# bcgsc/RNA-Bloom

Hardware: AMD Instinct MI355X
Metric: k-mers/sec hashed+inserted into Bloom dBG (k=25, 50M 150bp reads) (higher is better)
Workload: dtype u64

## Files before the change

### rna-bloom_amd/csrc/rb_capi.hip

```cpp
#include <math.h>
#include <stdarg.h>
#include <stdlib.h>
#include <string.h>
#include <time.h>

#include <algorithm>
#include <new>
#include <vector>

#include <functional>
#include <string>
#include <thread>

#include <fcntl.h>
#include <unistd.h>
#include <zlib.h>

#include "rb_pipeline.hpp"

using namespace rb;

namespace {

__global__ void k_popcount_bits(const uint32_t *__restrict__ w, size_t n_words, unsigned long long *out) {
// ... 652 lines not shown
            size_t m = std::min(chunk, n - done);
            g->keys0.reserve(m * 8); g->vals0.reserve(m * 4);
            RB_HIP(hipMemcpyAsync(g->keys0.p, h0 + done, m * 8, hipMemcpyHostToDevice, s));
            hipLaunchKernelGGL(k_iota, dim3(blocks_for((int64_t)m)), dim3(TPB), 0, s, g->vals0.as<uint32_t>(), m);
            run_pipeline(g, m, mode, g->ordinal, 0, nullptr);
            g->ordinal += m;
            done += m;
        }
        RB_HIP(hipStreamSynchronize(s));
    });
}

}
namespace {
__global__ void k_debug_probe(uint32_t *words, uint64_t n_words, uint32_t per_thread, int mode, uint64_t salt, unsigned long long *sink) {
    const uint64_t t = (uint64_t)blockIdx.x * blockDim.x + threadIdx.x;
    uint64_t x = (t + salt) * 0x9E3779B97F4A7C15ull + 0x632BE59BD9B4E019ull;
    uint32_t acc = 0;
    for (uint32_t i = 0; i < per_thread; ++i) {
        x ^= x >> 30; x *= 0xBF58476D1CE4E5B9ull; x ^= x >> 27; x *= 0x94D049BB133111EBull; x ^= x >> 31;
        uint32_t *w = &words[(uint64_t)(((unsigned __int128)x * n_words) >> 64)];
        acc |= mode ? atomicXor(w, 0x80808080u) : atomicOr(w, 0u);
    }
    if (acc == 0x12345678u) atomicAdd(sink, 1ull);
}
}
extern "C" {
int rb_debug_probe_cbf(rb_graph *g, int mode, float *ms_out) {
    return guarded([&] {
        RB_REQUIRE(g && g->cbf && ms_out, "rb_debug_probe_cbf: bad argument");
        rb::WriteLock wl(g->rw);
        RB_HIP(hipSetDevice(g->p.device));
        hipStream_t s = g->stream;
        g->devctr.reserve(DEVCTR_BYTES);
        rb::Event e0, e1;
        RB_HIP(hipEventCreate(&e0.e)); RB_HIP(hipEventCreate(&e1.e));
        RB_HIP(hipStreamSynchronize(s));
        RB_HIP(hipEventRecord(e0, s));
        for (int pass = 0; pass < 2; ++pass)
            hipLaunchKernelGGL(k_debug_probe, dim3(65536), dim3(256), 0, s, reinterpret_cast<uint32_t *>(g->cbf), (uint64_t)(g->cbf_alloc / 4), 16u, mode, 0ull, g->devctr.as<unsigned long long>());
        RB_HIP(hipEventRecord(e1, s));
        RB_HIP(hipEventSynchronize(e1));
        RB_HIP(hipEventElapsedTime(ms_out, e0, e1));
    });
}

int rb_debug_scan_u32(int device, const uint32_t *in, size_t n, uint32_t *out, int misalign) {
    DevBuf a, b, t;
    return guarded([&] {
        RB_REQUIRE((in && out) || n == 0, "rb_debug_scan_u32: null array");
        RB_REQUIRE(misalign >= 0 && misalign < 16, "rb_debug_scan_u32: misalign in 0..15");
        RB_HIP(hipSetDevice(device));
        a.reserve((n + 8) * 4); b.reserve((n + 8) * 4); t.reserve(scan_temp_bytes(n));
        uint32_t *di = a.as<uint32_t>() + (misalign & 3), *dout = b.as<uint32_t>() + ((misalign >> 2) & 3);
        if (n) RB_HIP(hipMemcpy(di, in, n * 4, hipMemcpyHostToDevice));
        exclusive_scan_u32(t.p, t.cap, di, dout, n, nullptr);
        RB_HIP(hipGetLastError());
        RB_HIP(hipDeviceSynchronize());
        if (n) RB_HIP(hipMemcpy(out, dout, n * 4, hipMemcpyDeviceToHost));
    });
}
int rb_debug_sort_pairs(int device, uint64_t *keys, void *vals, int vals64, size_t n, int lo_begin, int lo_end, int hi_begin, int hi_end) {
    DevBuf k0, k1, v0, v1, t;
    return guarded([&] {
        RB_REQUIRE(keys || n == 0, "rb_debug_sort_pairs: null keys");
        RB_REQUIRE(!(vals64 && hi_begin >= 0), "rb_debug_sort_pairs: two ranges with 32-bit values only");
        RB_HIP(hipSetDevice(device));
        if (n == 0) return;
        const size_t vb = vals64 ? 8 : 4;
        k0.reserve(n * 8); k1.reserve(n * 8);
        if (vals) { v0.reserve(n * vb); v1.reserve(n * vb); RB_HIP(hipMemcpy(v0.p, vals, n * vb, hipMemcpyHostToDevice)); }
        RB_HIP(hipMemcpy(k0.p, keys, n * 8, hipMemcpyHostToDevice));
        t.reserve(vals64 ? sort_pairs32_temp_bytes(n) : sort_pairs_temp_bytes(n));
        if (vals64) sort_pairs_u64_u64(t.p, t.cap, k0.as<uint64_t>(), k1.as<uint64_t>(), v0.as<uint64_t>(), v1.as<uint64_t>(), n, lo_begin, lo_end, nullptr);
        else if (hi_begin >= 0) sort_pairs_u64_u32_2r(t.p, t.cap, k0.as<uint64_t>(), k1.as<uint64_t>(), v0.as<uint32_t>(), v1.as<uint32_t>(), n, lo_begin, lo_end, hi_begin, hi_end, nullptr);
        else if (vals) sort_pairs_u64_u32(t.p, t.cap, k0.as<uint64_t>(), k1.as<uint64_t>(), v0.as<uint32_t>(), v1.as<uint32_t>(), n, lo_begin, lo_end, nullptr);
        else sort_keys_u64(t.p, t.cap, k0.as<uint64_t>(), k1.as<uint64_t>(), n, lo_begin, lo_end, nullptr);
        RB_HIP(hipGetLastError());
        RB_HIP(hipDeviceSynchronize());
        RB_HIP(hipMemcpy(keys, k1.p, n * 8, hipMemcpyDeviceToHost));
        if (vals) RB_HIP(hipMemcpy(vals, v1.p, n * vb, hipMemcpyDeviceToHost));
    });
}
int rb_filter_size(rb_graph *g, int which, int64_t *size, int64_t *nbytes, int *num_hash) {
    if (!g) { set_error("null graph"); return RB_ERR_INVALID; }
    if (which == RB_CBF) {
        if (!g->cbf) { set_error("rb_filter_size: filter %d not initialised", which); return RB_ERR_STATE; }
        if (size) *size = g->cbf_size;
        if (nbytes) *nbytes = g->cbf_hi - g->cbf_lo;
        if (num_hash) *num_hash = g->cbf_h;
        return RB_OK;
    }
    BitFilter *f = bit_filter(g, which);
    if (!f) { set_error("rb_filter_size: unknown filter %d", which); return RB_ERR_INVALID; }
    if (!f->bits) { set_error("rb_filter_size: filter %d not initialised", which); return RB_ERR_STATE; }
    if (size) *size = f->size;
    if (nbytes) *nbytes = f->nbytes;
    if (num_hash) *num_hash = f->num_hash;
    return RB_OK;
}

static int filter_reduce(rb_graph *g, int which, bool fold, unsigned long long *out) {
    return guarded([&] {
        RB_REQUIRE(g && out, "rb_filter_popcount / rb_filter_fold: null argument");
        QueryLease q(g);
        RB_HIP(hipStreamSynchronize(g->stream));
        q.c->b0.reserve(64);
        unsigned long long *acc = q.c->b0.as<unsigned long long>();
        RB_HIP(hipMemsetAsync(acc, 0, 8, q.c->st));
        const uint32_t *words; size_t nw; uint64_t gw0;
        if (which == RB_CBF) {
            if (!g->cbf) { set_error("rb_filter_popcount: filter %d not initialised", which); throw HipError{RB_ERR_STATE}; }
            words = reinterpret_cast<const uint32_t *>(g->cbf); nw = g->cbf_alloc / 4;
            gw0 = (uint64_t)g->cbf_lo / 4u;
        } else {
            BitFilter *f = bit_filter(g, which);
            RB_REQUIRE(f, "rb_filter_popcount: unknown filter %d", which);
            if (!f->bits) { set_error("rb_filter_popcount: filter %d not initialised", which); throw HipError{RB_ERR_STATE}; }
            words = f->bits; nw = f->alloc / 4;
            gw0 = (uint64_t)f->lo / 32u;
        }
        const dim3 grid(std::min<unsigned>(blocks_for((int64_t)nw), 8192u));
        if (fold) hipLaunchKernelGGL(k_fold_words, grid, dim3(TPB), 0, q.c->st, words, nw, gw0, acc);
        else if (which == RB_CBF) hipLaunchKernelGGL(k_count_nonzero_bytes, grid, dim3(TPB), 0, q.c->st, words, nw, acc);
        else hipLaunchKernelGGL(k_popcount_bits, grid, dim3(TPB), 0, q.c->st, words, nw, acc);
        RB_HIP(hipGetLastError());
        unsigned long long v = 0;
        RB_HIP(hipMemcpyAsync(&v, acc, 8, hipMemcpyDeviceToHost, q.c->st));
        RB_HIP(hipStreamSynchronize(q.c->st));
        *out = v;
    });
}
int rb_filter_popcount(rb_graph *g, int which, int64_t *out) {
    unsigned long long v = 0;
    if (!out) { set_error("rb_filter_popcount: null argument"); return RB_ERR_INVALID; }
    int rc = filter_reduce(g, which, false, &v);
    if (rc == RB_OK) *out = (int64_t)v;
    return rc;
}
int rb_filter_fold(rb_graph *g, int which, uint64_t *out) {
    unsigned long long v = 0;
    if (!out) { set_error("rb_filter_fold: null argument"); return RB_ERR_INVALID; }
    int rc = filter_reduce(g, which, true, &v);
    if (rc == RB_OK) *out = (uint64_t)v;
    return rc;
}

int rb_filter_fpr(rb_graph *g, int which, float *out) {
    int64_t pop = 0, size = 0; int h = 0;
    int rc = rb_filter_popcount(g, which, &pop);
    if (rc != RB_OK) return rc;
    rc = rb_filter_size(g, which, &size, nullptr, &h);
    if (rc != RB_OK) return rc;
    if (!out) { set_error("null argument"); return RB_ERR_INVALID; }
    *out = (float)pow((double)pop / (double)size, h);
    return RB_OK;
}

int rb_filter_export(rb_graph *g, int which, void *dst, size_t nbytes) {
    return guarded([&] {
        RB_REQUIRE(g && dst, "rb_filter_export: null argument");
        QueryLease q(g);
        const void *src; size_t have;
        if (which == RB_CBF) { src = g->cbf; have = (size_t)(g->cbf_hi - g->cbf_lo); }
        else {
            BitFilter *f = bit_filter(g, which);
// ... 123 lines not shown
```

### rna-bloom_amd/csrc/rb_group.hip

```cpp
#include <stdlib.h>

#include <algorithm>

#include "rb_pipeline.hpp"

namespace rb {

constexpr uint32_t GR_KEY_TOP = 60;
constexpr uint32_t GR_MAX_GROUP_BITS = 36;
constexpr uint32_t GR_TILE = 4096;
constexpr uint32_t GR_BUCKET_TARGET = 3072;
constexpr uint32_t GR_LOCAL_BITS = 8;
constexpr uint32_t GR_PART_MAX_BITS = 10;

constexpr uint64_t GR_DEAD_KEY = ~0ull;
constexpr uint32_t GR_DEAD_VAL = ~0u;
__device__ __forceinline__ uint32_t gr_digit(uint64_t key, uint32_t shift, uint32_t bits) {
    return (uint32_t)(key >> shift) & ((1u << bits) - 1u);
}
struct GrIdxDev { Mod mod; uint64_t lo, mul; uint32_t top, shift; };
__device__ __forceinline__ uint32_t gr_idx_digit(uint64_t key, const GrIdxDev &ix, uint32_t bits) {
    const uint64_t i = index_of(key, ix.mod) - ix.lo;
    const uint32_t d = min((uint32_t)min(__umul64hi(i, ix.mul), (uint64_t)0xFFFFFFFFull), ix.top);
    return (d >> ix.shift) & ((1u << bits) - 1u);
// ... 51 lines not shown
template <int ITEMS, typename CT>
__device__ __forceinline__ void gr_wave_rank_lds_wide(const uint32_t (&dig)[ITEMS], uint32_t (&rank)[ITEMS], CT *wc, unsigned long long *wm, uint32_t bits,
                                                      uint32_t rows) {
    const uint32_t lane = threadIdx.x & 63u;
#pragma unroll
    for (int r = 0; r < ITEMS; ++r) {
        if ((uint32_t)r < rows) {
            const bool valid = dig[r] != ~0u;
            uint64_t ml = 0;
            uint32_t prior = 0;
            if (valid) {
                __hip_atomic_fetch_or(&wm[dig[r] & 255u], 1ull << lane, __ATOMIC_RELAXED, __HIP_MEMORY_SCOPE_WORKGROUP);
                ml = __hip_atomic_load(&wm[dig[r] & 255u], __ATOMIC_RELAXED, __HIP_MEMORY_SCOPE_WORKGROUP);
                prior = (uint32_t)wc[dig[r]];
            }
            uint64_t m = ml;
            for (uint32_t b = 8; b < bits; ++b) {
                const bool bit = valid && ((dig[r] >> b) & 1u);
                const uint64_t bal = __ballot(bit);
                m &= bit ? bal : ~bal;
            }
            rank[r] = prior + gr_lanes_below(m);
            if (valid && (ml >> lane) == 1ull) __hip_atomic_store(&wm[dig[r] & 255u], 0ull, __ATOMIC_RELAXED, __HIP_MEMORY_SCOPE_WORKGROUP);
            if (valid && (m >> lane) == 1ull) wc[dig[r]] = (CT)(prior + (uint32_t)__popcll(m));
            __builtin_amdgcn_wave_barrier();
        }
    }
}

template <int TPB>
__device__ __forceinline__ uint32_t gr_block_excl_scan(uint32_t v, uint32_t *s_wsum) {
    const uint32_t lane = threadIdx.x & 63u, w = threadIdx.x >> 6;
    uint32_t inc = v;
#pragma unroll
    for (int o = 1; o < 64; o <<= 1) {
        const uint32_t t = __shfl_up(inc, o, 64);
        if ((int)lane >= o) inc += t;
    }
    if (lane == 63u) s_wsum[w] = inc;
    __syncthreads();
    uint32_t base = 0;
#pragma unroll
    for (int i = 0; i < TPB / 64; ++i) {
        const uint32_t t = s_wsum[i];
        if ((uint32_t)i < w) base += t;
    }
    __syncthreads();
    return base + inc - v;
}

template <int TPB, typename CT, typename DT>
__device__ __forceinline__ void gr_digit_offsets(CT *wcnt , DT *dstart , uint32_t nb, uint32_t *s_wsum) {
    constexpr int NW = TPB / 64;
    const uint32_t per = (nb + TPB - 1) / TPB;
    uint32_t tot[4] = {0, 0, 0, 0}, sum = 0;
    for (uint32_t q = 0; q < per; ++q) {
        const uint32_t d = threadIdx.x * per + q;
        if (d < nb) {
            uint32_t run = 0;
#pragma unroll
            for (int w = 0; w < NW; ++w) { const uint32_t t = (uint32_t)wcnt[(uint32_t)w * nb + d]; wcnt[(uint32_t)w * nb + d] = (CT)run; run += t; }
            tot[q] = run; sum += run;
        }
    }
    uint32_t base = gr_block_excl_scan<TPB>(sum, s_wsum);
    for (uint32_t q = 0; q < per; ++q) {
        const uint32_t d = threadIdx.x * per + q;
        if (d < nb) { dstart[d] = (DT)base; base += tot[q]; }
    }
}

__device__ __forceinline__ uint32_t gr_tile_of_block(uint32_t b, uint32_t grid_tiles, int xcd_map) {
    if (!xcd_map) return b;
    return (b & 7u) * (grid_tiles >> 3) + (b >> 3);
}
inline uint32_t gr_grid_for_tiles(uint32_t ntiles) { return ((ntiles + 7u) / 8u) * 8u; }

struct GrTile { uint32_t start, count, hist_base, hist_stride; };
struct GrTiling {
    const GrTile *desc;
    const uint32_t *ntiles_dev;
    uint32_t n, ntiles, grid_tiles;
    int xcd_map;
};
__device__ __forceinline__ bool gr_get_tile(const GrTiling &tl, GrTile &t) {
    const uint32_t i = gr_tile_of_block(blockIdx.x, tl.grid_tiles, tl.xcd_map);
    if (!tl.desc) {
        if (i >= tl.ntiles) return false;
        t.start = i * GR_TILE; t.count = min(GR_TILE, tl.n - t.start); t.hist_base = i; t.hist_stride = tl.ntiles;
        return true;
    }
    if (i >= *tl.ntiles_dev) return false;
    t = tl.desc[i];
    return true;
}

template <int TPB, bool DERIVE = false>
__global__ void __launch_bounds__(TPB) k_part_count(const uint64_t *__restrict__ keys, GrTiling tl, uint32_t shift, uint32_t bits,
                                                    uint32_t *__restrict__ hist, const uint32_t *__restrict__ dead_vals = nullptr,
                                                    GrIdxDev ix = GrIdxDev{Mod{1, 0, 0}, 0, 0, 0, 0}, uint64_t kmul = 0) {
    constexpr int ITEMS = GR_TILE / TPB;
    __shared__ uint32_t s_h[1u << GR_PART_MAX_BITS];
    GrTile t;
    if (!gr_get_tile(tl, t)) return;
    const uint32_t nb = 1u << bits;
    for (uint32_t d = threadIdx.x; d < nb; d += TPB) s_h[d] = 0;
    __syncthreads();
    uint64_t k[ITEMS];
#pragma unroll
    for (int i = 0; i < ITEMS; ++i) {
        const uint32_t j = (uint32_t)i * TPB + threadIdx.x;
        k[i] = j < t.count ? keys[t.start + j] : 0ull;
        if (DERIVE) k[i] = multi_hash(k[i], 1u, kmul);
    }
#pragma unroll
    for (int i = 0; i < ITEMS; ++i) {
        const uint32_t j = (uint32_t)i * TPB + threadIdx.x;
        if (j < t.count && !(dead_vals && k[i] == GR_DEAD_KEY && dead_vals[t.start + j] == GR_DEAD_VAL))
            atomicAdd(&s_h[ix.mul ? gr_idx_digit(k[i], ix, bits) : gr_digit(k[i], shift, bits)], 1u);
    }
    __syncthreads();
    for (uint32_t d = threadIdx.x; d < nb; d += TPB) hist[(size_t)t.hist_base + (size_t)d * t.hist_stride] = s_h[d];
}

template <int TPB, int MAXBITS, bool DERIVE = false>
__global__ void __launch_bounds__(TPB) k_part_scatter(const uint64_t *__restrict__ keys_in, const uint32_t *__restrict__ vals_in, GrTiling tl,
                                                      uint32_t shift, uint32_t bits, const uint32_t *__restrict__ goffs ,
                                                      uint64_t *__restrict__ keys_out, uint32_t *__restrict__ vals_out, uint32_t wide_lds,
                                                      uint32_t skip_dead = 0u, GrIdxDev ix = GrIdxDev{Mod{1, 0, 0}, 0, 0, 0, 0}, uint64_t kmul = 0) {
    constexpr uint32_t ITEMS = GR_TILE / TPB, NW = TPB / 64, SEG = 64 * ITEMS, MAXNB = 1u << MAXBITS;
    __shared__ uint64_t s_keys[GR_TILE];
    __shared__ uint32_t s_vals[GR_TILE];
    __shared__ uint32_t s_cnt[NW * MAXNB / 2 > MAXNB ? NW * MAXNB / 2 : MAXNB];
    __shared__ uint16_t s_dstart[MAXNB];
    __shared__ uint32_t s_wsum[NW];
    constexpr bool NARROW = MAXBITS <= 8;
    static_assert(sizeof(s_vals) >= NW * 256u * sizeof(unsigned long long), "the mask table must fit the staging array");
    unsigned long long *s_wmask = reinterpret_cast<unsigned long long *>(s_vals);
    uint16_t *s_wcnt = reinterpret_cast<uint16_t *>(s_cnt);
    GrTile t;
    if (!gr_get_tile(tl, t)) return;
    const uint32_t nb = 1u << bits;
    const uint32_t w = threadIdx.x >> 6, lane = threadIdx.x & 63u;
    for (uint32_t d = threadIdx.x; d < NW * nb; d += TPB) s_wcnt[d] = 0;
    for (uint32_t d = threadIdx.x; d < NW * (NARROW ? nb : 256u); d += TPB) s_wmask[d] = 0ull;
    uint64_t k[ITEMS];
    uint32_t v[ITEMS], dig[ITEMS], rank[ITEMS];
#pragma unroll
    for (uint32_t r = 0; r < ITEMS; ++r) {
        const uint32_t j = w * SEG + r * 64u + lane;
        bool ok = j < t.count;
        k[r] = ok ? keys_in[t.start + j] : 0ull;
        v[r] = (ok && vals_in) ? vals_in[t.start + j] : 0u;
        if (DERIVE) { k[r] = multi_hash(k[r], 1u, kmul); v[r] = t.start + j; }
        if (skip_dead && k[r] == GR_DEAD_KEY && v[r] == GR_DEAD_VAL) ok = false;
        dig[r] = ok ? (ix.mul ? gr_idx_digit(k[r], ix, bits) : gr_digit(k[r], shift, bits)) : ~0u;
    }
    const uint32_t rows = t.count > w * SEG ? min(ITEMS, (t.count - w * SEG + 63u) / 64u) : 0u;
    __syncthreads();
    if (NARROW) gr_wave_rank_lds<ITEMS>(dig, rank, s_wcnt + w * nb, s_wmask + w * nb, rows);
    else if (wide_lds) gr_wave_rank_lds_wide<ITEMS>(dig, rank, s_wcnt + w * nb, s_wmask + w * 256u, bits, rows);
    else gr_wave_rank<ITEMS>(dig, rank, s_wcnt + w * nb, bits, rows);
    __syncthreads();
    gr_digit_offsets<TPB>(s_wcnt, s_dstart, nb, s_wsum);
    __syncthreads();
#pragma unroll
    for (uint32_t r = 0; r < ITEMS; ++r)
        if (dig[r] != ~0u) {
            const uint32_t p = (uint32_t)s_dstart[dig[r]] + (uint32_t)s_wcnt[w * nb + dig[r]] + rank[r];
            s_keys[p] = k[r]; s_vals[p] = v[r];
        }
    __syncthreads();
    uint32_t live = 0;
#pragma unroll
    for (uint32_t i = 0; i < NW; ++i) live += s_wsum[i];
    for (uint32_t d = threadIdx.x; d < nb; d += TPB) s_cnt[d] = goffs[(size_t)t.hist_base + (size_t)d * t.hist_stride] - (uint32_t)s_dstart[d];
    __syncthreads();
    for (uint32_t j = threadIdx.x; j < live; j += TPB) {
        const uint64_t key = s_keys[j];
        const uint32_t g = s_cnt[ix.mul ? gr_idx_digit(key, ix, bits) : gr_digit(key, shift, bits)] + j;
        keys_out[g] = key;
        if (vals_out) vals_out[g] = s_vals[j];
    }
}

__global__ void __launch_bounds__(1024) k_seg_tiles(const uint32_t *__restrict__ goffs1, uint32_t ntiles1, uint32_t nb1, uint32_t n, uint32_t nb2,
                                                    GrTile *__restrict__ desc, uint32_t *__restrict__ seg_tile_base ,
                                                    uint32_t *__restrict__ seg_start , uint32_t *__restrict__ ntiles2_dev,
                                                    const uint32_t *__restrict__ n_dev = nullptr ) {
    __shared__ uint32_t s_wsum[16];
    const uint32_t b = threadIdx.x;
    if (n_dev) n = *n_dev;
    uint32_t s = 0, e = 0;
    if (b < nb1) { s = goffs1[(size_t)b * ntiles1]; e = b + 1u < nb1 ? goffs1[(size_t)(b + 1u) * ntiles1] : n; }
    const uint32_t nt = (e - s + GR_TILE - 1u) / GR_TILE;
    const uint32_t tb = gr_block_excl_scan<1024>(nt, s_wsum);
    if (b < nb1) {
        seg_tile_base[b] = tb; seg_start[b] = s;
        for (uint32_t i = 0; i < nt; ++i) {
            GrTile t; t.start = s + i * GR_TILE; t.count = min(GR_TILE, e - t.start); t.hist_base = tb * nb2 + i; t.hist_stride = nt;
            desc[tb + i] = t;
        }
        if (b == nb1 - 1u) { seg_tile_base[nb1] = tb + nt; seg_start[nb1] = n; *ntiles2_dev = tb + nt; }
    }
}
// ... 444 lines not shown
    int xcd_map = 1;
    size_t hist_entries = 0;
    size_t off_status = 0, off_ticket = 0, off_bstart = 0, off_big = 0, off_hist = 0, off_goffs = 0, off_scan = 0, off_desc = 0, off_segtb = 0, off_segst = 0,
           scan_bytes = 0, total = 0;
};
static size_t gr_align(size_t x) { return (x + 255) / 256 * 256; }

static GroupPlan group_plan(size_t N, int group_bits, int bucket_target = 0, int flags = 0, int force_T = -1) {
    GroupPlan P;
    P.n = (uint32_t)N;
    P.dead = (flags & GR_FLAG_DEAD) != 0;
    const uint32_t gb = (uint32_t)std::max(1, std::min<int>(group_bits, (int)GR_MAX_GROUP_BITS));
    uint32_t T = 0;
    const size_t target = getenv("RB_GROUP_TARGET") ? (size_t)std::max(64, std::min(atoi(getenv("RB_GROUP_TARGET")), (int)GR_TILE))
                        : bucket_target > 0 ? (size_t)bucket_target : (size_t)GR_BUCKET_TARGET;
    while ((target << T) < N) ++T;
    if (const char *e = getenv("RB_GROUP_T")) T = (uint32_t)std::max(0, atoi(e));
    if (force_T >= 0) T = (uint32_t)force_T;
    T = std::min({T, gb, 2u * GR_PART_MAX_BITS});
    if (P.dead && T == 0) T = 1;
    P.T = T;
    if (T <= GR_PART_MAX_BITS) { P.t_hi = T; P.t_lo = 0; }
    else { P.t_hi = (T + 1u) / 2u; P.t_lo = T - P.t_hi; }
    P.shift_hi = GR_KEY_TOP - P.t_hi;
    P.shift_lo = GR_KEY_TOP - T;
    const uint32_t L = std::min(gb - T, 2u * GR_LOCAL_BITS);
    P.l_hi = (L + 1u) / 2u;
    P.l_lo = L - P.l_hi;
    P.lshift_hi = GR_KEY_TOP - T - P.l_hi;
    P.lshift_lo = GR_KEY_TOP - T - L;
    P.tpb = getenv("RB_GROUP_TPB") ? (uint32_t)atoi(getenv("RB_GROUP_TPB")) : 512u;
    if (P.tpb != 256u) P.tpb = 512u;
    P.xcd_map = getenv("RB_GROUP_XCD") ? atoi(getenv("RB_GROUP_XCD")) : 1;
    P.fix_cap = L == 2u * GR_LOCAL_BITS ? (bucket_target > 0 ? 2u : 1u) : 0u;
    if (const char *e = getenv("RB_GROUP_FIX")) P.fix_cap = (uint32_t)std::max(0, std::min(atoi(e), 2));
    P.ntiles = (uint32_t)((N + GR_TILE - 1) / GR_TILE);
    P.ntiles2_max = P.t_lo ? P.ntiles + (1u << P.t_hi) : 0;
    P.nbuckets = 1u << T;
    if (T) P.hist_entries = std::max((size_t)P.ntiles << P.t_hi, (size_t)P.ntiles2_max << P.t_lo) + 2;
    size_t o = 0;
    P.off_status = o; o += gr_align((size_t)P.nbuckets * 8);
    P.off_ticket = o; o += 256;
    P.off_bstart = o; o += gr_align(((size_t)P.nbuckets + 1) * 4);
    P.off_big = o; o += gr_align((size_t)P.nbuckets * 4);
    if (T) {
        P.off_hist = o; o += gr_align(P.hist_entries * 4);
        P.off_goffs = o; o += gr_align(P.hist_entries * 4);
        P.scan_bytes = gr_align(scan_temp_bytes(P.hist_entries));
        P.off_scan = o; o += P.scan_bytes;
        if (P.t_lo) {
            P.off_desc = o; o += gr_align((size_t)P.ntiles2_max * sizeof(GrTile));
            P.off_segtb = o; o += gr_align(((size_t)(1u << P.t_hi) + 1) * 4);
            P.off_segst = o; o += gr_align(((size_t)(1u << P.t_hi) + 1) * 4);
        }
    }
    P.total = o;
    return P;
}

void group_debug_big(const void *temp, size_t N, int group_bits, int bucket_target, uint32_t *n_big_out, uint64_t *records_out, uint32_t *largest_out, int flags) {
    const GroupPlan P = group_plan(N, group_bits, bucket_target, flags);
    const char *tp = static_cast<const char *>(temp);
    uint32_t tick[4] = {0, 0, 0, 0};
    RB_HIP(hipMemcpy(tick, tp + P.off_ticket, 16, hipMemcpyDeviceToHost));
    const uint32_t nb = std::min(tick[2], P.nbuckets);
    std::vector<uint32_t> big(nb), bs((size_t)P.nbuckets + 1);
    if (nb) RB_HIP(hipMemcpy(big.data(), tp + P.off_big, (size_t)nb * 4, hipMemcpyDeviceToHost));
    RB_HIP(hipMemcpy(bs.data(), tp + P.off_bstart, ((size_t)P.nbuckets + 1) * 4, hipMemcpyDeviceToHost));
    uint64_t rec = 0; uint32_t mx = 0;
    for (uint32_t i = 0; i < nb; ++i) { const uint32_t c = bs[big[i] + 1] - bs[big[i]]; rec += c; mx = std::max(mx, c); }
    *n_big_out = nb; *records_out = rec; *largest_out = mx;
}
size_t group_temp_bytes(size_t N, int group_bits, int bucket_target, int flags) { return group_plan(N, group_bits, bucket_target, flags).total; }
const uint32_t *group_live_count(const void *temp, size_t N, int group_bits, int bucket_target, int flags) {
    const GroupPlan P = group_plan(N, group_bits, bucket_target, flags);
    return reinterpret_cast<const uint32_t *>(static_cast<const char *>(temp) + P.off_ticket) + 3;
}

template <int TPB>
static void part_pass(const GrTiling &tl, size_t entries, uint32_t shift, uint32_t bits, const uint64_t *kin, const uint32_t *vin, uint64_t *kout,
                      uint32_t *vout, uint32_t *hist, uint32_t *goffs, void *scan_tmp, size_t scan_bytes, hipStream_t st, rb_graph *prof,
                      uint32_t *n_live_dev = nullptr ,
                      GrIdxDev ix = GrIdxDev{Mod{1, 0, 0}, 0, 0, 0, 0}, uint64_t derive_kmul = 0 ) {
    const dim3 grid(tl.grid_tiles), blk(TPB);
    if (prof) prof->prof_begin(st);
    if (n_live_dev) RB_HIP(hipMemsetAsync(hist + entries, 0, 4, st));
    if (derive_kmul) hipLaunchKernelGGL((k_part_count<TPB, true>), grid, blk, 0, st, kin, tl, shift, bits, hist, (const uint32_t *)nullptr, ix, derive_kmul);
    else hipLaunchKernelGGL(k_part_count<TPB>, grid, blk, 0, st, kin, tl, shift, bits, hist, n_live_dev ? vin : (const uint32_t *)nullptr, ix);
    if (prof) { prof->prof_end("group_part_count", st); prof->prof_begin(st); }
    exclusive_scan_u32(scan_tmp, scan_bytes, hist, goffs, entries + (n_live_dev ? 1 : 0), st);
    if (n_live_dev) hipLaunchKernelGGL(k_copy_u32, dim3(1), dim3(64), 0, st, n_live_dev, goffs + entries);
    if (prof) { prof->prof_end("group_scan", st); prof->prof_begin(st); }
    const uint32_t wide = !(getenv("RB_GROUP_WIDE_LDS") && atoi(getenv("RB_GROUP_WIDE_LDS")) == 0);
    if (derive_kmul) {
        if (bits <= 8u) hipLaunchKernelGGL((k_part_scatter<TPB, 8, true>), grid, blk, 0, st, kin, (const uint32_t *)nullptr, tl, shift, bits, goffs, kout, vout, wide, 0u, ix, derive_kmul);
        else hipLaunchKernelGGL((k_part_scatter<TPB, GR_PART_MAX_BITS, true>), grid, blk, 0, st, kin, (const uint32_t *)nullptr, tl, shift, bits, goffs, kout, vout, wide, 0u, ix, derive_kmul);
    } else if (bits <= 8u) hipLaunchKernelGGL((k_part_scatter<TPB, 8>), grid, blk, 0, st, kin, vin, tl, shift, bits, goffs, kout, vout, wide, n_live_dev ? 1u : 0u, ix);
    else hipLaunchKernelGGL((k_part_scatter<TPB, GR_PART_MAX_BITS>), grid, blk, 0, st, kin, vin, tl, shift, bits, goffs, kout, vout, wide, n_live_dev ? 1u : 0u, ix);
    if (prof) prof->prof_end("group_part_scatter", st);
}

namespace {
struct LsdPlan {
    uint32_t ntiles = 0, n_pass = 0, shift[16], bits[16];
    size_t entries = 0, off_hist = 0, off_goffs = 0, off_scan = 0, scan_bytes = 0, off_idx = 0, total = 0;
};
LsdPlan lsd_plan(size_t n, const int (*ranges)[2], int n_ranges, bool idx_vals) {
    LsdPlan P;
    P.ntiles = (uint32_t)((n + GR_TILE - 1) / GR_TILE);
    uint32_t maxbits = 0;
    for (int r = 0; r < n_ranges; ++r) {
        const uint32_t B = (uint32_t)std::max(0, ranges[r][1] - ranges[r][0]);
        const uint32_t maxb = n <= ((size_t)1 << 20) ? 8u : GR_PART_MAX_BITS;
        const uint32_t np = (B + maxb - 1) / maxb;
        uint32_t lo = (uint32_t)ranges[r][0], left = B;
        for (uint32_t q = 0; q < np; ++q) {
            const uint32_t b = (left + (np - q) - 1) / (np - q);
            P.shift[P.n_pass] = lo; P.bits[P.n_pass] = b; ++P.n_pass;
            lo += b; left -= b;
            maxbits = std::max(maxbits, b);
        }
    }
    P.entries = ((size_t)P.ntiles << maxbits) + 2;
    size_t o = 0;
    P.off_hist = o; o += gr_align(P.entries * 4);
    P.off_goffs = o; o += gr_align(P.entries * 4);
    P.scan_bytes = gr_align(scan_temp_bytes(P.entries));
    P.off_scan = o; o += P.scan_bytes;
    if (idx_vals) { P.off_idx = o; o += 2 * gr_align(n * 4); }
    P.total = o;
    return P;
}
void lsd_sort(const LsdPlan &P, char *tp, uint64_t *k_in, uint64_t *k_out, uint32_t *v_in, uint32_t *v_out, size_t n, hipStream_t st) {
    uint32_t *hist = reinterpret_cast<uint32_t *>(tp + P.off_hist), *goffs = reinterpret_cast<uint32_t *>(tp + P.off_goffs);
    const GrTiling tl{nullptr, nullptr, (uint32_t)n, P.ntiles, gr_grid_for_tiles(P.ntiles), 1};
    uint64_t *ka = k_in, *kb = k_out;
    uint32_t *va = v_in, *vb = v_out;
    for (uint32_t q = 0; q < P.n_pass; ++q) {
        part_pass<512>(tl, (size_t)P.ntiles << P.bits[q], P.shift[q], P.bits[q], ka, va, kb, vb, hist, goffs, tp + P.off_scan, P.scan_bytes, st, nullptr);
        std::swap(ka, kb); std::swap(va, vb);
    }
    if ((P.n_pass & 1u) == 0) {
        RB_HIP(hipMemcpyAsync(k_out, k_in, n * 8, hipMemcpyDeviceToDevice, st));
        if (v_in && v_out) RB_HIP(hipMemcpyAsync(v_out, v_in, n * 4, hipMemcpyDeviceToDevice, st));
    }
}
__global__ void k_lsd_iota(uint32_t *__restrict__ v, size_t n) {
    const size_t i = (size_t)blockIdx.x * blockDim.x + threadIdx.x;
    if (i < n) v[i] = (uint32_t)i;
}
__global__ void k_lsd_gather64(const uint32_t *__restrict__ idx, const uint64_t *__restrict__ src, uint64_t *__restrict__ dst, size_t n) {
    const size_t i = (size_t)blockIdx.x * blockDim.x + threadIdx.x;
    if (i < n) dst[i] = src[idx[i]];
}
}

size_t sort_pairs_temp_bytes(size_t n) { const int r[1][2] = {{0, 64}}; return lsd_plan(n, r, 1, false).total; }
size_t sort_keys_temp_bytes(size_t n) { return sort_pairs_temp_bytes(n); }
size_t sort_pairs32_temp_bytes(size_t n) { const int r[1][2] = {{0, 64}}; return lsd_plan(n, r, 1, true).total; }
void sort_pairs_u64_u32(void *temp, size_t temp_bytes, uint64_t *keys_in, uint64_t *keys_out, uint32_t *vals_in, uint32_t *vals_out, size_t n,
                        int begin_bit, int end_bit, hipStream_t s) {
    if (n == 0) return;
    RB_REQUIRE(n < (1ull << 32) - 2 * GR_TILE, "sort_pairs_u64_u32: too many records");
    const int r[1][2] = {{begin_bit, end_bit}};
    const LsdPlan P = lsd_plan(n, r, 1, false);
    RB_REQUIRE(temp_bytes >= P.total, "sort_pairs_u64_u32: temp too small");
    lsd_sort(P, static_cast<char *>(temp), keys_in, keys_out, vals_in, vals_out, n, s);
}
void sort_pairs_u64_u32_2r(void *temp, size_t temp_bytes, uint64_t *keys_in, uint64_t *keys_out, uint32_t *vals_in, uint32_t *vals_out, size_t n,
                           int lo_begin, int lo_end, int hi_begin, int hi_end, hipStream_t s) {
    if (n == 0) return;
    RB_REQUIRE(n < (1ull << 32) - 2 * GR_TILE, "sort_pairs_u64_u32_2r: too many records");
    const int r[2][2] = {{lo_begin, lo_end}, {hi_begin, hi_end}};
    const LsdPlan P = lsd_plan(n, r, 2, false);
    RB_REQUIRE(temp_bytes >= P.total, "sort_pairs_u64_u32_2r: temp too small");
    lsd_sort(P, static_cast<char *>(temp), keys_in, keys_out, vals_in, vals_out, n, s);
}
void sort_keys_u64(void *temp, size_t temp_bytes, uint64_t *keys_in, uint64_t *keys_out, size_t n, int begin_bit, int end_bit, hipStream_t s) {
    sort_pairs_u64_u32(temp, temp_bytes, keys_in, keys_out, nullptr, nullptr, n, begin_bit, end_bit, s);
}
void sort_pairs_u64_u64(void *temp, size_t temp_bytes, uint64_t *keys_in, uint64_t *keys_out, uint64_t *vals_in, uint64_t *vals_out, size_t n,
                        int begin_bit, int end_bit, hipStream_t s) {
    if (n == 0) return;
    RB_REQUIRE(n < (1ull << 32) - 2 * GR_TILE, "sort_pairs_u64_u64: too many records");
    const int r[1][2] = {{begin_bit, end_bit}};
    const LsdPlan P = lsd_plan(n, r, 1, true);
    RB_REQUIRE(temp_bytes >= P.total, "sort_pairs_u64_u64: temp too small");
    char *tp = static_cast<char *>(temp);
    uint32_t *i0 = reinterpret_cast<uint32_t *>(tp + P.off_idx), *i1 = reinterpret_cast<uint32_t *>(tp + P.off_idx + gr_align(n * 4));
    hipLaunchKernelGGL(k_lsd_iota, dim3((unsigned)((n + 255) / 256)), dim3(256), 0, s, i0, n);
    lsd_sort(P, tp, keys_in, keys_out, i0, i1, n, s);
    hipLaunchKernelGGL(k_lsd_gather64, dim3((unsigned)((n + 255) / 256)), dim3(256), 0, s, i1, vals_in, vals_out, n);
}

static GrIdxDev gr_idx_dev(const GroupPlan &P, const GrIdx &idx) {
    if (idx.span > (1ull << P.T))
        return GrIdxDev{idx.mod, idx.lo, (uint64_t)((((unsigned __int128)1 << 64) << P.T) / idx.span), (1u << P.T) - 1u, P.t_lo};
    return GrIdxDev{Mod{1, 0, 0}, 0, 0, 0, 0};
}
template <int TPB>
static uint32_t *partition_records(const GroupPlan &P, uint64_t *keys0, uint32_t *vals0, uint64_t *keys_tmp, uint32_t *vals_tmp, char *tp, hipStream_t st,
                                   rb_graph *prof, GrIdx idx, const uint64_t **kin_out, const uint32_t **vin_out,
                                   const uint64_t *derive_src = nullptr, uint64_t derive_kmul = 0 ) {
    unsigned long long *status = reinterpret_cast<unsigned long long *>(tp + P.off_status);
    uint32_t *ticket = reinterpret_cast<uint32_t *>(tp + P.off_ticket);
    uint32_t *bstart = reinterpret_cast<uint32_t *>(tp + P.off_bstart);
    RB_HIP(hipMemsetAsync(status, 0, P.off_bstart, st));
    const uint64_t *kin = derive_src ? derive_src : keys0;
    const uint32_t *vin = derive_src ? nullptr : vals0;
    if (P.T) {
        uint32_t *hist = reinterpret_cast<uint32_t *>(tp + P.off_hist), *goffs = reinterpret_cast<uint32_t *>(tp + P.off_goffs);
        void *scan_tmp = tp + P.off_scan;
        GrTiling t1{nullptr, nullptr, P.n, P.ntiles, gr_grid_for_tiles(P.ntiles), P.xcd_map};
        uint32_t *n_live = P.dead ? ticket + 3 : nullptr;
        GrIdxDev ix = gr_idx_dev(P, idx);
        part_pass<TPB>(t1, (size_t)P.ntiles << P.t_hi, P.shift_hi, P.t_hi, kin, vin, keys_tmp, vals_tmp, hist, goffs, scan_tmp, P.scan_bytes, st, prof, n_live, ix, derive_src ? derive_kmul : 0);
        kin = keys_tmp; vin = vals_tmp;
        uint32_t *segtb = nullptr, *segst = nullptr;
        if (P.t_lo) {
            GrTile *desc = reinterpret_cast<GrTile *>(tp + P.off_desc);
            segtb = reinterpret_cast<uint32_t *>(tp + P.off_segtb); segst = reinterpret_cast<uint32_t *>(tp + P.off_segst);
            uint32_t *nt2 = ticket + 1;
            hipLaunchKernelGGL(k_seg_tiles, dim3(1), dim3(1024), 0, st, goffs, P.ntiles, 1u << P.t_hi, P.n, 1u << P.t_lo, desc, segtb, segst, nt2, (const uint32_t *)n_live);
            RB_HIP(hipMemsetAsync(hist, 0, ((size_t)P.ntiles2_max << P.t_lo) * 4, st));
            GrTiling t2{desc, nt2, P.n, P.ntiles2_max, gr_grid_for_tiles(P.ntiles2_max), P.xcd_map};
            ix.shift = 0;
            part_pass<TPB>(t2, (size_t)P.ntiles2_max << P.t_lo, P.shift_lo, P.t_lo, kin, vin, keys0, vals0, hist, goffs, scan_tmp, P.scan_bytes, st, prof, nullptr, ix);
            kin = keys0; vin = vals0;
        }
        hipLaunchKernelGGL(k_bucket_bounds, dim3((P.nbuckets + 256u) / 256u), dim3(256), 0, st, goffs, P.ntiles, segtb, segst, P.t_hi, P.t_lo, P.n, bstart, (const uint32_t *)n_live);
    } else
        hipLaunchKernelGGL(k_bucket_bounds, dim3(1), dim3(64), 0, st, (const uint32_t *)nullptr, 0u, (const uint32_t *)nullptr, (const uint32_t *)nullptr, 0u, 0u, P.n, bstart);
    *kin_out = kin; *vin_out = vin;
    return bstart;
}

template <int TPB>
static void group_records_impl(const GroupPlan &P, uint64_t *keys0, uint32_t *vals0, uint64_t *keys_tmp, uint32_t *vals_tmp, GroupRng rng, char *tp,
                               uint32_t *vals_out, uint8_t *tz_out, uint64_t *uniq, uint32_t *counts, uint32_t *starts, uint32_t *n_runs_dev,
                               hipStream_t st, rb_graph *prof, GrIdx idx, GroupExport ex) {
    unsigned long long *status = reinterpret_cast<unsigned long long *>(tp + P.off_status);
    uint32_t *ticket = reinterpret_cast<uint32_t *>(tp + P.off_ticket);
    const uint64_t *kin = nullptr;
    const uint32_t *vin = nullptr;
    uint32_t *bstart = partition_records<TPB>(P, keys0, vals0, keys_tmp, vals_tmp, tp, st, prof, idx, &kin, &vin);
    uint32_t *big_list = reinterpret_cast<uint32_t *>(tp + P.off_big), *n_big = ticket + 2;
    if (prof) prof->prof_begin(st);
    const uint32_t bucket_grid = std::min(P.nbuckets, (uint32_t)(getenv("RB_GROUP_GRID") ? atoi(getenv("RB_GROUP_GRID")) : 768));
    const bool ordered = getenv("RB_GROUP_ORDERED") && atoi(getenv("RB_GROUP_ORDERED")) != 0;
    if (!ordered) RB_HIP(hipMemsetAsync(n_runs_dev, 0, 4, st));
    const bool prefetch = !(getenv("RB_GROUP_PREFETCH") && atoi(getenv("RB_GROUP_PREFETCH")) == 0);
    const uint32_t by_class = getenv("RB_GROUP_CLASSES") ? (uint32_t)(atoi(getenv("RB_GROUP_CLASSES")) != 0) : 1u;
    if (ordered || !prefetch)
        hipLaunchKernelGGL((k_group_buckets<TPB, false>), dim3(bucket_grid), dim3(TPB), 0, st, kin, vin, bstart, P.nbuckets, P.lshift_lo, P.l_lo, P.lshift_hi, P.l_hi,
                           rng, P.fix_cap, ticket, ordered ? status : nullptr, big_list, n_big, vals_out, tz_out, uniq, counts, starts, n_runs_dev, 0u, ex.brun, ex.bnr);
    else
        hipLaunchKernelGGL((k_group_buckets<TPB, true>), dim3(bucket_grid), dim3(TPB), 0, st, kin, vin, bstart, P.nbuckets, P.lshift_lo, P.l_lo, P.lshift_hi, P.l_hi,
                           rng, P.fix_cap, ticket, nullptr, big_list, n_big, vals_out, tz_out, uniq, counts, starts, n_runs_dev, by_class, ex.brun, ex.bnr);
    if (ex.n_main) hipLaunchKernelGGL(k_copy_u32, dim3(1), dim3(64), 0, st, ex.n_main, n_runs_dev);
    if (prof) { prof->prof_end("group_buckets", st); prof->prof_begin(st); }
    uint64_t *ka = const_cast<uint64_t *>(kin), *kb = kin == keys0 ? keys_tmp : keys0;
    uint32_t *va = const_cast<uint32_t *>(vin), *vb = vin == vals0 ? vals_tmp : vals0;
    hipLaunchKernelGGL(k_group_big<512>, dim3(std::min(P.nbuckets, 2048u)), dim3(512), 0, st, ka, va, kb, vb, bstart, big_list, n_big,
                       P.lshift_lo, P.l_lo, P.lshift_hi, P.l_hi, rng, vals_out, tz_out, uniq, counts, starts, n_runs_dev);
    if (prof) prof->prof_end("group_big_buckets", st);
    RB_HIP(hipGetLastError());
}

void group_records_device(uint64_t *keys0, uint32_t *vals0, uint64_t *keys_tmp, uint32_t *vals_tmp, size_t N, int group_bits,
                          uint64_t seed, uint64_t ordinal0, uint32_t pos_bits, void *temp, size_t temp_bytes,
                          uint32_t *vals_out, uint8_t *tz_out, uint64_t *uniq, uint32_t *counts, uint32_t *starts, uint32_t *n_runs_dev,
                          hipStream_t st, rb_graph *prof, int bucket_target, int flags, GrIdx idx, GroupExport ex) {
    RB_REQUIRE(N > 0 && N < (1ull << 32) - 2 * GR_TILE, "group_records_device: bad record count");
    const GroupPlan P = group_plan(N, group_bits, bucket_target, flags);
    RB_REQUIRE(temp_bytes >= P.total, "group_records_device: temp too small");
    const GroupRng rng{seed, ordinal0, pos_bits};
    if (P.tpb == 512u) group_records_impl<512>(P, keys0, vals0, keys_tmp, vals_tmp, rng, static_cast<char *>(temp), vals_out, tz_out, uniq, counts, starts, n_runs_dev, st, prof, idx, ex);
    else group_records_impl<256>(P, keys0, vals0, keys_tmp, vals_tmp, rng, static_cast<char *>(temp), vals_out, tz_out, uniq, counts, starts, n_runs_dev, st, prof, idx, ex);
}
uint32_t group_index_buckets(size_t N, int group_bits, int bucket_target, int flags, GrIdx idx) {
    const GroupPlan P = group_plan(N, group_bits, bucket_target, flags);
    return (P.T && idx.span > (1ull << P.T)) ? P.T : 0u;
}

constexpr uint32_t SW_WORDS = 16384;
constexpr uint32_t SW_MARKS = 1024;
__device__ __forceinline__ uint32_t sw_digit(uint64_t x, const GrIdxDev &ix) {
    return min((uint32_t)min(__umul64hi(x, ix.mul), (uint64_t)0xFFFFFFFFull), ix.top);
}
__device__ __forceinline__ uint64_t sw_first(uint32_t c, const GrIdxDev &ix, uint64_t span, uint32_t T) {
    if (c == 0u) return 0ull;
    if (c > ix.top) return span;
    uint64_t e = ((uint64_t)c * span) >> T;
    while (e > 0ull && sw_digit(e - 1ull, ix) >= c) --e;
    while (e < span && sw_digit(e, ix) < c) ++e;
    return e;
}
template <int TPB>
__global__ void __launch_bounds__(TPB, 4) k_sweep_bits(uint32_t *words, GrIdxDev ix, uint64_t span, uint32_t T, const uint64_t *__restrict__ uniq,
                                                    const uint32_t *__restrict__ brun, const uint32_t *__restrict__ bnr,
                                                    const uint64_t *__restrict__ k1, const uint32_t *__restrict__ v1, const uint32_t *__restrict__ bstart1,
                                                    uint8_t *st0, uint8_t *st1, uint32_t SWW ) {
    extern __shared__ __attribute__((aligned(16))) uint32_t sw_lds[];
    uint32_t *s_w = sw_lds, *s_c = sw_lds + SWW, *s_t = sw_lds + SWW + SW_MARKS;
    __shared__ uint32_t s_any;
    const uint32_t c = blockIdx.x;
    const uint32_t r0 = brun[c], nr = bnr[c], p0 = bstart1[c], p1 = bstart1[c + 1u];
    if (nr == 0u && p0 == p1) return;
// ... 130 lines not shown
```

Before: 39.68 billion.

## Count runs of tiles per block in partition histogram with packed 16-bit LDS counters

The partition-count kernel now has each block process a run of up to 16 consecutive tiles instead of one. The next tile's keys are prefetched while the current tile is counted, and per-tile histograms are packed as two 16-bit counters per LDS word. This cuts block launch and setup overhead and LDS footprint, and overlaps global loads with LDS atomics. The costs are a smaller grid with possibly lower occupancy, an environment-variable override, and a new test C API entry point.

```diff
diff --git a/rna-bloom_amd/csrc/rb_capi.hip b/rna-bloom_amd/csrc/rb_capi.hip
--- a/rna-bloom_amd/csrc/rb_capi.hip
+++ b/rna-bloom_amd/csrc/rb_capi.hip
@@ -758,6 +758,35 @@
         if (vals) RB_HIP(hipMemcpy(vals, v1.p, n * vb, hipMemcpyDeviceToHost));
     });
 }
+int rb_test_group_records(int device, const uint64_t *keys, const uint32_t *occ, size_t n, int group_bits, int bucket_target, int flags, uint64_t idx_size,
+                          uint64_t seed, uint64_t ordinal0, uint32_t pos_bits, uint32_t *occ_out, uint8_t *tz_out, uint64_t *uniq, uint32_t *counts,
+                          uint32_t *starts, uint32_t *n_runs, uint32_t *n_live) {
+    DevBuf k0, k1, v0, v1, t, vo, tz, u, c, s, nr;
+    return guarded([&] {
+        RB_REQUIRE(keys && occ && n > 0 && occ_out && tz_out && uniq && counts && starts && n_runs && n_live, "rb_test_group_records: bad argument");
+        RB_HIP(hipSetDevice(device));
+        k0.reserve(n * 8); k1.reserve(n * 8); v0.reserve(n * 4); v1.reserve(n * 4); vo.reserve(n * 4); tz.reserve(n + 16); u.reserve(n * 8);
+        c.reserve(n * 4 + 4); s.reserve(n * 4 + 4); nr.reserve(64);
+        t.reserve(group_temp_bytes(n, group_bits, bucket_target, flags));
+        RB_HIP(hipMemcpy(k0.p, keys, n * 8, hipMemcpyHostToDevice));
+        RB_HIP(hipMemcpy(v0.p, occ, n * 4, hipMemcpyHostToDevice));
+        const GrIdx idx = idx_size ? GrIdx{make_mod(idx_size), 0, idx_size} : GrIdx{Mod{1, 0, 0}, 0, 0};
+        group_records_device(k0.as<uint64_t>(), v0.as<uint32_t>(), k1.as<uint64_t>(), v1.as<uint32_t>(), n, group_bits, seed, ordinal0, pos_bits, t.p, t.cap,
+                             vo.as<uint32_t>(), tz.as<uint8_t>(), u.as<uint64_t>(), c.as<uint32_t>(), s.as<uint32_t>(), nr.as<uint32_t>(), nullptr, nullptr,
+                             bucket_target, flags, idx);
+        RB_HIP(hipGetLastError());
+        RB_HIP(hipDeviceSynchronize());
+        *n_live = (uint32_t)n;
+        if (flags & GR_FLAG_DEAD) RB_HIP(hipMemcpy(n_live, group_live_count(t.p, n, group_bits, bucket_target, flags), 4, hipMemcpyDeviceToHost));
+        RB_HIP(hipMemcpy(n_runs, nr.p, 4, hipMemcpyDeviceToHost));
+        RB_REQUIRE(*n_runs <= n && *n_live <= n, "rb_test_group_records: %u runs, %u live of %zu records", *n_runs, *n_live, n);
+        RB_HIP(hipMemcpy(occ_out, vo.p, (size_t)*n_live * 4, hipMemcpyDeviceToHost));
+        RB_HIP(hipMemcpy(tz_out, tz.p, (size_t)*n_live, hipMemcpyDeviceToHost));
+        RB_HIP(hipMemcpy(uniq, u.p, (size_t)*n_runs * 8, hipMemcpyDeviceToHost));
+        RB_HIP(hipMemcpy(counts, c.p, (size_t)*n_runs * 4, hipMemcpyDeviceToHost));
+        RB_HIP(hipMemcpy(starts, s.p, (size_t)*n_runs * 4, hipMemcpyDeviceToHost));
+    });
+}
 int rb_filter_size(rb_graph *g, int which, int64_t *size, int64_t *nbytes, int *num_hash) {
     if (!g) { set_error("null graph"); return RB_ERR_INVALID; }
     if (which == RB_CBF) {
diff --git a/rna-bloom_amd/csrc/rb_group.hip b/rna-bloom_amd/csrc/rb_group.hip
--- a/rna-bloom_amd/csrc/rb_group.hip
+++ b/rna-bloom_amd/csrc/rb_group.hip
@@ -157,45 +157,89 @@
     const uint32_t *ntiles_dev;
     uint32_t n, ntiles, grid_tiles;
     int xcd_map;
+    uint32_t run_log2, grid_runs;
 };
+__device__ __forceinline__ GrTile gr_uniform_tile(const GrTiling &tl, uint32_t i) {
+    GrTile t;
+    t.start = i * GR_TILE; t.count = min(GR_TILE, tl.n - t.start); t.hist_base = i; t.hist_stride = tl.ntiles;
+    return t;
+}
 __device__ __forceinline__ bool gr_get_tile(const GrTiling &tl, GrTile &t) {
     const uint32_t i = gr_tile_of_block(blockIdx.x, tl.grid_tiles, tl.xcd_map);
     if (!tl.desc) {
         if (i >= tl.ntiles) return false;
-        t.start = i * GR_TILE; t.count = min(GR_TILE, tl.n - t.start); t.hist_base = i; t.hist_stride = tl.ntiles;
+        t = gr_uniform_tile(tl, i);
         return true;
     }
     if (i >= *tl.ntiles_dev) return false;
     t = tl.desc[i];
     return true;
 }
-
+constexpr uint32_t GR_RUN_MAX_LOG2 = 4, GR_RUN_MIN_GRID = 1024;
+inline void gr_set_runs(GrTiling &tl) {
+    uint32_t lg = GR_RUN_MAX_LOG2;
+    while (lg > 0 && ((tl.ntiles + (1u << lg) - 1u) >> lg) < GR_RUN_MIN_GRID) --lg;
+    if (const char *e = getenv("RB_GROUP_RUN")) { const int g = atoi(e); lg = 0; while (lg < GR_RUN_MAX_LOG2 && (2 << lg) <= g) ++lg; }
+    tl.run_log2 = lg;
+    tl.grid_runs = gr_grid_for_tiles((tl.ntiles + (1u << lg) - 1u) >> lg);
+}
+
+constexpr uint32_t GR_COL_WORDS = (1u << GR_PART_MAX_BITS) / 2u + 1u;
 template <int TPB, bool DERIVE = false>
 __global__ void __launch_bounds__(TPB) k_part_count(const uint64_t *__restrict__ keys, GrTiling tl, uint32_t shift, uint32_t bits,
                                                     uint32_t *__restrict__ hist, const uint32_t *__restrict__ dead_vals = nullptr,
                                                     GrIdxDev ix = GrIdxDev{Mod{1, 0, 0}, 0, 0, 0, 0}, uint64_t kmul = 0) {
     constexpr int ITEMS = GR_TILE / TPB;
-    __shared__ uint32_t s_h[1u << GR_PART_MAX_BITS];
-    GrTile t;
-    if (!gr_get_tile(tl, t)) return;
-    const uint32_t nb = 1u << bits;
-    for (uint32_t d = threadIdx.x; d < nb; d += TPB) s_h[d] = 0;
-    __syncthreads();
-    uint64_t k[ITEMS];
+    static_assert(TPB % (1 << GR_RUN_MAX_LOG2) == 0, "a thread writes out the entries of ONE tile of the run");
+    __shared__ uint32_t s_h[GR_COL_WORDS << GR_RUN_MAX_LOG2];
+    __shared__ GrTile s_tile[1u << GR_RUN_MAX_LOG2];
+    const uint32_t G = 1u << tl.run_log2;
+    const uint32_t i0 = gr_tile_of_block(blockIdx.x, tl.grid_runs, tl.xcd_map) << tl.run_log2;
+    const uint32_t ntiles = tl.desc ? *tl.ntiles_dev : tl.ntiles;
+    if (i0 >= ntiles) return;
+    const uint32_t cnt = min(G, ntiles - i0);
+    const uint32_t nb = 1u << bits, colw = nb / 2u + 1u;
+    for (uint32_t d = threadIdx.x; d < colw * cnt; d += TPB) s_h[d] = 0;
+    if (threadIdx.x < cnt) s_tile[threadIdx.x] = tl.desc ? tl.desc[i0 + threadIdx.x] : gr_uniform_tile(tl, i0 + threadIdx.x);
+    __syncthreads();
+    uint64_t k[ITEMS], kn[ITEMS];
+    uint32_t start = __builtin_amdgcn_readfirstlane(s_tile[0].start), count = __builtin_amdgcn_readfirstlane(s_tile[0].count);
 #pragma unroll
     for (int i = 0; i < ITEMS; ++i) {
         const uint32_t j = (uint32_t)i * TPB + threadIdx.x;
-        k[i] = j < t.count ? keys[t.start + j] : 0ull;
-        if (DERIVE) k[i] = multi_hash(k[i], 1u, kmul);
-    }
-#pragma unroll
-    for (int i = 0; i < ITEMS; ++i) {
-        const uint32_t j = (uint32_t)i * TPB + threadIdx.x;
-        if (j < t.count && !(dead_vals && k[i] == GR_DEAD_KEY && dead_vals[t.start + j] == GR_DEAD_VAL))
-            atomicAdd(&s_h[ix.mul ? gr_idx_digit(k[i], ix, bits) : gr_digit(k[i], shift, bits)], 1u);
-    }
-    __syncthreads();
-    for (uint32_t d = threadIdx.x; d < nb; d += TPB) hist[(size_t)t.hist_base + (size_t)d * t.hist_stride] = s_h[d];
+        kn[i] = j < count ? keys[start + j] : 0ull;
+    }
+    for (uint32_t g = 0; g < cnt; ++g) {
+        const uint32_t t_start = start, t_count = count;
+#pragma unroll
+        for (int i = 0; i < ITEMS; ++i) k[i] = kn[i];
+        if (g + 1u < cnt) {
+            start = __builtin_amdgcn_readfirstlane(s_tile[g + 1u].start); count = __builtin_amdgcn_readfirstlane(s_tile[g + 1u].count);
+#pragma unroll
+            for (int i = 0; i < ITEMS; ++i) {
+                const uint32_t j = (uint32_t)i * TPB + threadIdx.x;
+                kn[i] = j < count ? keys[start + j] : 0ull;
+            }
+        }
+        uint32_t *col = s_h + g * colw;
+#pragma unroll
+        for (int i = 0; i < ITEMS; ++i) {
+            const uint32_t j = (uint32_t)i * TPB + threadIdx.x;
+            if (DERIVE) k[i] = multi_hash(k[i], 1u, kmul);
+            if (j < t_count && !(dead_vals && k[i] == GR_DEAD_KEY && dead_vals[t_start + j] == GR_DEAD_VAL)) {
+                const uint32_t d = ix.mul ? gr_idx_digit(k[i], ix, bits) : gr_digit(k[i], shift, bits);
+                atomicAdd(&col[d >> 1], 1u << ((d & 1u) << 4));
+            }
+        }
+    }
+    __syncthreads();
+    const uint32_t g = threadIdx.x & (G - 1u);
+    if (g < cnt) {
+        const GrTile t = s_tile[g];
+        const uint32_t *col = s_h + g * colw;
+        for (uint32_t d = threadIdx.x >> tl.run_log2; d < nb; d += TPB >> tl.run_log2)
+            hist[(size_t)t.hist_base + (size_t)d * t.hist_stride] = (col[d >> 1] >> ((d & 1u) << 4)) & 0xFFFFu;
+    }
 }
 
 template <int TPB, int MAXBITS, bool DERIVE = false>
@@ -806,11 +850,11 @@
                       uint32_t *vout, uint32_t *hist, uint32_t *goffs, void *scan_tmp, size_t scan_bytes, hipStream_t st, rb_graph *prof,
                       uint32_t *n_live_dev = nullptr ,
                       GrIdxDev ix = GrIdxDev{Mod{1, 0, 0}, 0, 0, 0, 0}, uint64_t derive_kmul = 0 ) {
-    const dim3 grid(tl.grid_tiles), blk(TPB);
+    const dim3 grid(tl.grid_tiles), grid_runs(tl.grid_runs), blk(TPB);
     if (prof) prof->prof_begin(st);
     if (n_live_dev) RB_HIP(hipMemsetAsync(hist + entries, 0, 4, st));
-    if (derive_kmul) hipLaunchKernelGGL((k_part_count<TPB, true>), grid, blk, 0, st, kin, tl, shift, bits, hist, (const uint32_t *)nullptr, ix, derive_kmul);
-    else hipLaunchKernelGGL(k_part_count<TPB>, grid, blk, 0, st, kin, tl, shift, bits, hist, n_live_dev ? vin : (const uint32_t *)nullptr, ix);
+    if (derive_kmul) hipLaunchKernelGGL((k_part_count<TPB, true>), grid_runs, blk, 0, st, kin, tl, shift, bits, hist, (const uint32_t *)nullptr, ix, derive_kmul);
+    else hipLaunchKernelGGL(k_part_count<TPB>, grid_runs, blk, 0, st, kin, tl, shift, bits, hist, n_live_dev ? vin : (const uint32_t *)nullptr, ix);
     if (prof) { prof->prof_end("group_part_count", st); prof->prof_begin(st); }
     exclusive_scan_u32(scan_tmp, scan_bytes, hist, goffs, entries + (n_live_dev ? 1 : 0), st);
     if (n_live_dev) hipLaunchKernelGGL(k_copy_u32, dim3(1), dim3(64), 0, st, n_live_dev, goffs + entries);
@@ -857,7 +901,8 @@
 }
 void lsd_sort(const LsdPlan &P, char *tp, uint64_t *k_in, uint64_t *k_out, uint32_t *v_in, uint32_t *v_out, size_t n, hipStream_t st) {
     uint32_t *hist = reinterpret_cast<uint32_t *>(tp + P.off_hist), *goffs = reinterpret_cast<uint32_t *>(tp + P.off_goffs);
-    const GrTiling tl{nullptr, nullptr, (uint32_t)n, P.ntiles, gr_grid_for_tiles(P.ntiles), 1};
+    GrTiling tl{nullptr, nullptr, (uint32_t)n, P.ntiles, gr_grid_for_tiles(P.ntiles), 1, 0, 0};
+    gr_set_runs(tl);
     uint64_t *ka = k_in, *kb = k_out;
     uint32_t *va = v_in, *vb = v_out;
     for (uint32_t q = 0; q < P.n_pass; ++q) {
@@ -935,7 +980,8 @@
     if (P.T) {
         uint32_t *hist = reinterpret_cast<uint32_t *>(tp + P.off_hist), *goffs = reinterpret_cast<uint32_t *>(tp + P.off_goffs);
         void *scan_tmp = tp + P.off_scan;
-        GrTiling t1{nullptr, nullptr, P.n, P.ntiles, gr_grid_for_tiles(P.ntiles), P.xcd_map};
+        GrTiling t1{nullptr, nullptr, P.n, P.ntiles, gr_grid_for_tiles(P.ntiles), P.xcd_map, 0, 0};
+        gr_set_runs(t1);
         uint32_t *n_live = P.dead ? ticket + 3 : nullptr;
         GrIdxDev ix = gr_idx_dev(P, idx);
         part_pass<TPB>(t1, (size_t)P.ntiles << P.t_hi, P.shift_hi, P.t_hi, kin, vin, keys_tmp, vals_tmp, hist, goffs, scan_tmp, P.scan_bytes, st, prof, n_live, ix, derive_src ? derive_kmul : 0);
@@ -947,7 +993,8 @@
             uint32_t *nt2 = ticket + 1;
             hipLaunchKernelGGL(k_seg_tiles, dim3(1), dim3(1024), 0, st, goffs, P.ntiles, 1u << P.t_hi, P.n, 1u << P.t_lo, desc, segtb, segst, nt2, (const uint32_t *)n_live);
             RB_HIP(hipMemsetAsync(hist, 0, ((size_t)P.ntiles2_max << P.t_lo) * 4, st));
-            GrTiling t2{desc, nt2, P.n, P.ntiles2_max, gr_grid_for_tiles(P.ntiles2_max), P.xcd_map};
+            GrTiling t2{desc, nt2, P.n, P.ntiles2_max, gr_grid_for_tiles(P.ntiles2_max), P.xcd_map, 0, 0};
+            gr_set_runs(t2);
             ix.shift = 0;
             part_pass<TPB>(t2, (size_t)P.ntiles2_max << P.t_lo, P.shift_lo, P.t_lo, kin, vin, keys0, vals0, hist, goffs, scan_tmp, P.scan_bytes, st, prof, nullptr, ix);
             kin = keys0; vin = vals0;
```

After: 39.56 billion. About the same (-0.3%).
